# WangWen-Believer/DR-SLAM

Hardware: AMD Instinct MI355X
Metric: RGB-D frames/sec (extract+match) at 640x480 (higher is better)
Workload: dtype u8; 1 GPU; 640x480 synthetic RGB-D (TUM3 intrinsics), ORB extract 1000/1.2/8/20/7 + SearchByProjection(frame k, frame k-1, th=15) on consecutive frames; BASELINE config 2; batch_per_gpu=512, batches_in_flight_per_gpu=3, distinct_resident_input_batches_per_gpu=3, sequence_frames_per_rank=64

## Files before the change

### dr_slam_amd/csrc/capi.cpp

```cpp
#include "drfe_internal.h"
#include "map_upkeep_internal.h"
#include "triangulate_internal.h"
#include "sim3_internal.h"
#include "pnp_internal.h"
#include "init_internal.h"
#include "line3d_internal.h"
#include "pose_opt_internal.h"
#include "trans_opt_internal.h"
#include "sim3_opt_internal.h"
#include <atomic>
#include "post_internal.h"
#include "match_internal.h"
#include "planes_internal.h"
#include "bow_internal.h"
#include "lines_internal.h"

#include <algorithm>
#include <cstdlib>
#include <cstring>
#include <sched.h>
#include <cstdio>
#include <thread>
#include <new>

// ... 77 lines not shown
        hipError_t e = hipDeviceGetStreamPriorityRange(&prLow, &prHigh);
        if (e != hipSuccess) return e;
        static const int split = [] { const char* m = std::getenv("DRFE_LONG_PRIO"); return !m ? 0 : (m[0] == 's' && m[1] == 'p') ? 1 : (m[0] == 'l' ? 2 : 0); }();
        const int mid = (prLow + prHigh) / 2;
        return hipStreamCreateWithPriority(s, hipStreamNonBlocking, (mid != prLow && ((part == 1 && split == 1) || (part == 0 && split == 2))) ? mid : prLow);
    }
    int dev = 0, cus = 0;
    hipError_t e = hipGetDevice(&dev);
    if (e == hipSuccess) e = hipDeviceGetAttribute(&cus, hipDeviceAttributeMultiprocessorCount, dev);
    if (e != hipSuccess) return e;
    std::vector<uint32_t> mask((size_t)(cus + 31) / 32, 0u);
    const int cut = 32 * share / 100;
    for (int i = 0; i < cus; i++) {
        const bool first = (i % 32) < cut;
        if (first == (part == 0)) mask[(size_t)i / 32] |= 1u << (i % 32);
    }
    return hipExtStreamCreateWithCUMask(s, (uint32_t)mask.size(), mask.data());
}

static std::atomic<long long> g_poolCpuNs[3];
void drfe_pool_cpu_add(int pool, long long ns) { if (pool >= 0 && pool < 3) g_poolCpuNs[pool] += ns; }
extern "C" void drfe_debug_pool_cpu_ns(long long* out3) { for (int k = 0; k < 3; k++) out3[k] = g_poolCpuNs[k].exchange(0); }

extern "C" {

const char* drfe_version(void) { return "drfe 0.1 (gfx950)"; }

const char* drfe_last_error(const drfe_ctx* ctx) { return ctx ? ctx->err.c_str() : g_create_err.c_str(); }

void drfe_destroy(drfe_ctx* c)
{
    if (!c) return;
    (void)hipSetDevice(c->device);
    if (c->stream) (void)hipStreamSynchronize(c->stream);
    drfe_match_buffers_free(c);
    drfe_planes_free(c);
    drfe_bow_free(c);
    drfe_lines_free(c);
    drfe_cape_lanes_free(c);
    drfe_manhattan_free(c);
    drfe_plane_match_free(c);
    drfe_map_upkeep_free(c);
    drfe_triangulate_free(c);
    drfe_sim3_free(c);
    drfe_pnp_free(c);
    drfe_init_free(c);
    drfe_line3d_free(c);
    drfe_pose_opt_free(c);
    drfe_trans_opt_free(c);
    drfe_sim3_opt_free(c);
    drfe_post_free(c);
    drfe_one_shot_free(c);
    drfe_frame_lanes_free(c);
    void* ptrs[] = {c->d_geom, c->d_cells, c->d_tiles, c->d_taps, c->d_pattern, c->d_disc, c->d_pyr, c->d_blur,
                    c->d_cand0, c->d_cand1, c->d_node, c->d_candCount, c->d_sel, c->d_selCount, c->d_kps, c->d_kpsUn, c->d_desc,
                    c->d_kpCount, c->d_status, c->d_uRight, c->d_depth, c->d_gridOff, c->d_gridIdx, c->d_cellKp, c->d_cellDesc, c->d_match,
                    c->d_matchCount, c->d_poses, c->d_stage, c->d_callScratch, c->d_kpUV, c->d_kpDepth};
    for (void* p : ptrs)
        if (p) (void)hipFree(p);
    for (int i = 0; i < DRFE_STAGE_COUNT; i++)
        for (int j = 0; j < 2; j++)
            if (c->ev[i][j]) (void)hipEventDestroy(c->ev[i][j]);
    if (c->stream) (void)hipStreamDestroy(c->stream);
    delete c;
}

int drfe_create(const drfe_config* cfg, drfe_ctx** out)
{
    if (!cfg || !out) { g_create_err = "null argument"; return DRFE_ERR_INVALID; }
    *out = nullptr;
    if (cfg->nlevels < 1 || cfg->nlevels > DRFE_MAX_LEVELS || cfg->max_batch < 1 || cfg->nfeatures < 1 ||
        !(cfg->scale_factor > 1.0f) || cfg->max_width < 64 || cfg->max_height < 64 || cfg->max_width > 4095 ||
        cfg->max_height > 4095) {
        g_create_err = "invalid drfe_config";
        return DRFE_ERR_INVALID;
    }
    int ndev = 0;
    if (hipGetDeviceCount(&ndev) != hipSuccess || ndev <= 0) {
        g_create_err = "no HIP device: libdrfe has no CPU path";
        return DRFE_ERR_HIP;
    }
    if (cfg->device < 0 || cfg->device >= ndev) { g_create_err = "device ordinal out of range"; return DRFE_ERR_INVALID; }
    drfe_ctx* c = new (std::nothrow) drfe_ctx();
    if (!c) { g_create_err = "out of host memory"; return DRFE_ERR_INVALID; }
    c->cfg = *cfg;
    c->device = cfg->device;
    c->stream = nullptr;
    c->profile = false;
    c->lastBatch = 0;
    c->glueValid = false;
    c->mb = nullptr;
    c->ps = nullptr;
    c->planeLanes = nullptr;
    c->bow = nullptr;
    c->ls = nullptr;
    c->lsBatch = nullptr;
    c->capeLanes = nullptr;
    c->lsdDeviceGrow = 1;
    c->lsdRectMode = 0;
    c->capeBatch = nullptr;
    c->planesDeviceCape = 1;
    c->lsdDeviceNfa = 1;
    c->lsdStats[0] = c->lsdStats[1] = c->lsdStats[2] = c->lsdStats[3] = 0;
    c->capeStats[0] = c->capeStats[1] = 0;
    c->ahcStats[0] = c->ahcStats[1] = c->ahcStats[2] = c->ahcStats[3] = 0;
    c->planesDeviceVoxel = 1;
    c->planesDeviceRefit = 1;
    c->ahcRefitStats[0] = c->ahcRefitStats[1] = 0;
    c->planesDeviceAhc = 1;
    c->ahcArena = nullptr;
    c->lineWorkers = nullptr;
    c->frameLanes = nullptr;
    c->lineHost = nullptr;
    std::memset(&c->cam, 0, sizeof(c->cam));
    std::memset(&c->geom, 0, sizeof(c->geom));
    std::memset(c->ev, 0, sizeof(c->ev));
    std::memset(c->evUsed, 0, sizeof(c->evUsed));
    c->d_geom = nullptr; c->d_cells = nullptr; c->d_tiles = nullptr; c->d_taps = nullptr; c->d_pattern = nullptr;
    c->d_callScratch = nullptr; c->callScratchBytes = 0;
    c->d_disc = nullptr; c->d_pyr = nullptr; c->d_blur = nullptr; c->d_cand0 = nullptr; c->d_cand1 = nullptr;
    c->d_node = nullptr; c->d_candCount = nullptr; c->d_sel = nullptr; c->d_selCount = nullptr; c->d_kps = nullptr; c->d_kpsUn = nullptr; std::memset(&c->dist, 0, sizeof(c->dist));
    c->d_desc = nullptr; c->d_kpCount = nullptr; c->d_status = nullptr; c->d_uRight = nullptr; c->d_depth = nullptr;
    c->d_gridOff = nullptr; c->d_gridIdx = nullptr; c->d_cellKp = nullptr; c->d_cellDesc = nullptr; c->d_match = nullptr; c->d_matchCount = nullptr;
    c->d_poses = nullptr; c->d_stage = nullptr;

#define CREATE_FAIL(code)                 \
    do {                                  \
        g_create_err = c->err;            \
        drfe_destroy(c);                  \
        return (code);                    \
    } while (0)
#define CHIP(call)                                                                  \
    do {                                                                            \
        hipError_t e__ = (call);                                                    \
        if (e__ != hipSuccess) {                                                    \
            c->err = std::string(#call) + ": " + hipGetErrorString(e__);            \
            CREATE_FAIL(DRFE_ERR_HIP);                                              \
        }                                                                           \
    } while (0)

    CHIP(hipSetDevice(c->device));
    CHIP(hipStreamCreateWithFlags(&c->stream, hipStreamNonBlocking));
    for (int i = 0; i < DRFE_STAGE_COUNT; i++)
        for (int j = 0; j < 2; j++) CHIP(hipEventCreate(&c->ev[i][j]));
    drfe_build_tables(c);
    {
        const char* e = std::getenv("DRFE_FAST_GENERIC");
        c->fastGeneric = (e && e[0] == '1') ? 1 : 0;
        const char* es = std::getenv("DRFE_FAST_SCREEN");
        c->fastScreen = (es && es[0] >= '0' && es[0] <= '2') ? es[0] - '0' : 2;
        c->qtForceN = drfe_quadtree_parse_force(std::getenv("DRFE_QT_FORCE"), c->qtForce);
        const char* el = std::getenv("DRFE_LEVEL0_COPY");
        c->level0Copy = (el && el[0] == '1') ? 1 : 0;
        c->lastInPlace = 0;
        c->level0.assign((size_t)std::max(cfg->max_batch, 1), Level0Record{false, nullptr, 0});
    }

    DevGeom gmax;
    std::memset(&gmax, 0, sizeof(gmax));
    std::vector<FastCell> cells;
    std::vector<BlurTile> tiles;
    std::vector<ResizeTap> taps;
    int rc = drfe_build_geometry(c, cfg->max_width, cfg->max_height, &gmax, &cells, &tiles, &taps);
    if (rc != DRFE_OK) CREATE_FAIL(rc);
    const size_t B = (size_t)cfg->max_batch;
    c->pyrSlotBytesMax = (size_t)gmax.pyrSlotBytes;
    c->blurSlotBytesMax = (size_t)gmax.blurSlotBytes;
    c->candSlotElemsMax = (size_t)gmax.candSlotElems;
    c->maxKp = gmax.kpSlotElems;
    c->cellsCap = (int)cells.size() + 64;
    c->tilesCap = (int)tiles.size() + 64;
    c->tapsCap = (int)taps.size() + 64 + (cfg->nlevels >= 2 ? gmax.lv[1].rzBlocks + 64 : 0);
    const int nl = cfg->nlevels;

    CHIP(dalloc(&c->d_geom, 1));
    CHIP(dalloc(&c->d_cells, (size_t)c->cellsCap));
    CHIP(dalloc(&c->d_tiles, (size_t)c->tilesCap));
    CHIP(dalloc(&c->d_taps, (size_t)c->tapsCap));
    CHIP(dalloc(&c->d_pattern, 1024));
    CHIP(hipMemcpy(c->d_pattern, kPatternHost, 1024, hipMemcpyHostToDevice));
    {
        std::vector<int16_t> disc;
        for (int v = -DRFE_HALF_PATCH; v <= DRFE_HALF_PATCH; v++) {
            const int d = c->umax[v < 0 ? -v : v];
            for (int u = -d; u <= d; u++) { disc.push_back((int16_t)u); disc.push_back((int16_t)v); }
        }
        c->discCount = (int)disc.size() / 2;
        if (c->discCount > 12 * 64) { c->err = "IC_Angle disc exceeds 12 offsets per lane"; CREATE_FAIL(DRFE_ERR_INVALID); }
        CHIP(dalloc(&c->d_disc, disc.size()));
        CHIP(hipMemcpy(c->d_disc, disc.data(), disc.size() * sizeof(int16_t), hipMemcpyHostToDevice));
    }
    CHIP(dalloc(&c->d_pyr, B * c->pyrSlotBytesMax + 256));
    CHIP(dalloc(&c->d_blur, B * c->blurSlotBytesMax));
    CHIP(dalloc(&c->d_cand0, B * c->candSlotElemsMax));
    CHIP(dalloc(&c->d_cand1, B * c->candSlotElemsMax));
    CHIP(dalloc(&c->d_node, B * c->candSlotElemsMax));
    CHIP(dalloc(&c->d_candCount, B * DRFE_CC_SLOT));
    CHIP(dalloc(&c->d_sel, B * (size_t)c->maxKp));
    CHIP(dalloc(&c->d_selCount, B * nl));
    CHIP(dalloc(&c->d_kps, B * (size_t)c->maxKp));
    CHIP(dalloc(&c->d_desc, B * (size_t)c->maxKp * 32));
    CHIP(dalloc(&c->d_kpCount, B));
    CHIP(dalloc(&c->d_status, 4));
    CHIP(dalloc(&c->d_uRight, B * (size_t)c->maxKp));
    CHIP(dalloc(&c->d_depth, B * (size_t)c->maxKp));
    CHIP(dalloc(&c->d_gridOff, B * (DRFE_GRID_CELLS + 1)));
    CHIP(dalloc(&c->d_gridIdx, B * (size_t)c->maxKp));
    CHIP(dalloc(&c->d_cellKp, B * (size_t)c->maxKp));
    CHIP(dalloc(&c->d_cellDesc, B * (size_t)c->maxKp * 2));
    CHIP(dalloc(&c->d_match, B * (size_t)c->maxKp));
    CHIP(dalloc(&c->d_matchCount, B));
    CHIP(dalloc(&c->d_poses, 2 * B * 16));
    c->stageBytes = (size_t)cfg->max_width * cfg->max_height * 2;
    CHIP(dalloc(&c->d_stage, c->stageBytes));
    CHIP(hipMemset(c->d_kpCount, 0, sizeof(int) * B));
    CHIP(hipMemset(c->d_selCount, 0, sizeof(int) * B * nl));
    CHIP(hipMemset(c->d_status, 0, sizeof(int) * 4));
#undef CHIP
#undef CREATE_FAIL
    *out = c;
    return DRFE_OK;
}

int drfe_orb_scale_tables(const drfe_ctx* c, float* scale, float* inv_scale, float* sigma2, float* inv_sigma2)
{
    if (!c) return DRFE_ERR_INVALID;
    for (int i = 0; i < c->cfg.nlevels; i++) {
        if (scale) scale[i] = c->scale[i];
        if (inv_scale) inv_scale[i] = c->invScale[i];
        if (sigma2) sigma2[i] = c->sigma2[i];
        if (inv_sigma2) inv_sigma2[i] = c->invSigma2[i];
    }
    return DRFE_OK;
}

int drfe_orb_max_keypoints(const drfe_ctx* c) { return c ? c->maxKp : DRFE_ERR_INVALID; }

static int check_status(drfe_ctx* c)
{
    int st = 0;
    HIPCHK(c, hipMemcpy(&st, c->d_status, sizeof(int), hipMemcpyDeviceToHost));
    if (st & 1) { c->err = "FAST candidate arena overflow"; return DRFE_ERR_CAPACITY; }
    if (st & 2) { c->err = "quadtree node pool overflow"; return DRFE_ERR_CAPACITY; }
// ... 634 lines not shown
```

### dr_slam_amd/csrc/drfe_internal.h

```cpp
#ifndef DRFE_INTERNAL_H
#define DRFE_INTERNAL_H

#include <hip/hip_runtime.h>
#ifndef DRFE_NO_ROCTX
#include <roctracer/roctx.h>
#else
static inline int roctxRangePushA(const char*) { return 0; }
static inline int roctxRangePop() { return 0; }
#endif
#include <stdint.h>
#include <time.h>
#include <string>
#include <vector>

#include "../../include/drfe.h"
#include "../../include/drfe_debug.h"
#include "hip_buf.h"

#define DRFE_MAX_LEVELS 16
#define DRFE_EDGE 19
#define DRFE_HALF_PATCH 15
#define DRFE_GRID_COLS 64
#define DRFE_GRID_ROWS 48
#define DRFE_GRID_CELLS (DRFE_GRID_COLS * DRFE_GRID_ROWS)
// ... 51 lines not shown
    int inst[DRFE_MAX_LEVELS];
    int nlaunch;
    QtLaunch launch[DRFE_MAX_LEVELS];
};
int drfe_quadtree_design_load(int pixels);
void drfe_quadtree_plan(const DevGeom& g, int nframes, const int* force, int nforce, QtPlan* plan);
int drfe_quadtree_parse_force(const char* text, int* pairs);

#ifndef DRFE_CC_LINE
#define DRFE_CC_LINE 32
#endif
#define DRFE_CC_SLOT (DRFE_MAX_LEVELS * DRFE_CC_LINE)
#define DRFE_CC_IDX(slot, level) ((size_t)(slot) * DRFE_CC_SLOT + (size_t)(level) * DRFE_CC_LINE)

struct FastCell {
    uint16_t x0, y0;
    uint8_t ww, wh;
    uint8_t level, off;
    uint16_t offX, offY;
    uint32_t cellIdx;
    uint32_t srcOff;
    uint32_t pitch;
    uint32_t candOff, candCap;
    uint8_t ncp, nrb, rpl, pad;
    uint32_t ncpMagic;
};

struct BlurTile { uint16_t tx, ty; uint16_t level, pad; };

struct ResizeTap { uint16_t s0, s1; int16_t w0, w1; };

#include "undistort_math.h"
#include "level0_view.h"

struct Level0Record { bool inPlace; const uint8_t* frame; size_t rowStride; };

struct drfe_ctx {
    drfe_config cfg;
    int device;
    hipStream_t stream;
    std::string err;

    std::vector<float> scale, invScale, sigma2, invSigma2;
    std::vector<int> quota;
    int umax[DRFE_HALF_PATCH + 1];
    DevGeom geom;
    int maxKp;

    DevGeom* d_geom;
    FastCell* d_cells; int cellsCap;
    BlurTile* d_tiles; int tilesCap;
    ResizeTap* d_taps; int tapsCap;
    int8_t* d_pattern;
    int16_t* d_disc;
    int discCount;

    uint8_t* d_pyr; size_t pyrSlotBytesMax;
    uint8_t* d_blur; size_t blurSlotBytesMax;
    uint32_t* d_cand0; uint32_t* d_cand1; uint16_t* d_node; size_t candSlotElemsMax;
    int* d_candCount;
    uint32_t* d_sel;
    int* d_selCount;
    drfe_keypoint* d_kps;
    drfe_keypoint* d_kpsUn;
    DrfeDistortion dist;
    uint8_t* d_desc;
    int* d_kpCount;
    int* d_status;
    int fastScreen;
    int fastGeneric;
    int qtForce[2 * DRFE_MAX_LEVELS];
    int qtForceN = 0;
    int level0Copy;
    int lastInPlace;
    bool level0Staged = false;
    std::vector<Level0Record> level0;

    float* d_uRight; float* d_depth;
    int* d_gridOff; int* d_gridIdx;
    uint4* d_cellKp; uint4* d_cellDesc;
    int* d_match; int* d_matchCount;
    float* d_poses;
    uint8_t* d_stage;
    size_t stageBytes;
    uint32_t* d_kpUV;
    uint16_t* d_kpDepth;
    uint8_t* d_callScratch;
    size_t callScratchBytes;

    int lastBatch;
    bool glueValid;
    drfe_camera cam;

    struct MatchBuffers* mb;
    struct PlanesScratch* ps;
    std::vector<struct PlaneLane>* planeLanes;
    struct BowState* bow;
    struct LinesScratch* ls;
    struct LineHost* lineHost;
    struct OrbOneShot* oneShot;
    struct CapeScratch* cape;
    struct CapeBatchArena* capeBatch;
    int planesDeviceCape;
    std::vector<struct CapeLane>* capeLanes;
    struct SnBuffers* sn;
    struct MfBuffers* mf;
    struct PmBuffers* pm;
    struct MuBuffers* mu = nullptr;
// ... 70 lines not shown
    const char* last = static_cast<const char*>(p) + (bytes ? bytes - 1 : 0);
    if (hipPointerGetAttributes(&b, last) != hipSuccess) { (void)hipGetLastError(); return false; }
    return b.type == hipMemoryTypeHost;
}

static inline const char* drfe_stage_name(int stage)
{
    static const char* const names[DRFE_STAGE_COUNT] = {"drfe:pyramid", "drfe:fast", "drfe:quadtree", "drfe:blur", "drfe:orient+desc", "drfe:glue", "drfe:match", "drfe:fast_b"};
    return stage >= 0 && stage < DRFE_STAGE_COUNT ? names[stage] : "drfe:?";
}
static inline void prof_begin(drfe_ctx* c, int stage, hipStream_t s)
{
    (void)roctxRangePushA(drfe_stage_name(stage));
    if (c->profile) { (void)hipEventRecord(c->ev[stage][0], s); c->evUsed[stage] = true; }
}
static inline void prof_end(drfe_ctx* c, int stage, hipStream_t s)
{
    if (c->profile) (void)hipEventRecord(c->ev[stage][1], s);
    (void)roctxRangePop();
}
struct DrfeRange {
    explicit DrfeRange(const char* name) { (void)roctxRangePushA(name); }
    ~DrfeRange() { (void)roctxRangePop(); }
};

static inline hipError_t drfe_event_wait_sleeping(hipEvent_t ev)
{
    for (int spins = 0;; spins++) {
        const hipError_t e = hipEventQuery(ev);
        if (e != hipErrorNotReady) return e;
        if (spins < 4) continue;
        struct timespec ts = {0, spins < 40 ? 20000 : 100000};
        nanosleep(&ts, nullptr);
    }
}

void drfe_pool_cpu_add(int pool, long long ns);
struct DrfePoolCpuScope {
    int pool; struct timespec t0;
    explicit DrfePoolCpuScope(int p) : pool(p) { clock_gettime(CLOCK_THREAD_CPUTIME_ID, &t0); }
    ~DrfePoolCpuScope() { struct timespec t1; clock_gettime(CLOCK_THREAD_CPUTIME_ID, &t1); drfe_pool_cpu_add(pool, (t1.tv_sec - t0.tv_sec) * 1000000000LL + (t1.tv_nsec - t0.tv_nsec)); }
};

hipError_t drfe_long_kernel_stream(hipStream_t* s, int part);

int drfe_default_host_threads();
void drfe_cape_lanes_free(drfe_ctx* c);
void drfe_bow_slot_invalidate(drfe_ctx* c, int slot);
void drfe_bow_slots_invalidate(drfe_ctx* c, int first, int count);
void drfe_one_shot_free(drfe_ctx* c);
void drfe_frame_lanes_free(drfe_ctx* c);

int drfe_build_tables(drfe_ctx* c);
int drfe_build_geometry(drfe_ctx* c, int w, int h, DevGeom* g, std::vector<FastCell>* cells,
                        std::vector<BlurTile>* tiles, std::vector<ResizeTap>* taps);

hipError_t drfe_launch_orb(drfe_ctx* c, const uint8_t* d_gray, size_t frameStride, size_t rowStride, int nframes,
                           hipStream_t s, bool allowInPlace = false);
hipError_t drfe_launch_level0(drfe_ctx* c, const uint8_t* d_gray, size_t frameStride, size_t rowStride, int nframes, hipStream_t s);
void drfe_fastc_list_caps(const DevGeom& g, int caps[2]);
hipError_t drfe_launch_glue(drfe_ctx* c, const uint16_t* d_depth, size_t frameStride, size_t rowStride,
                            const drfe_camera& cam, int nframes, hipStream_t s);
hipError_t drfe_launch_grid(drfe_ctx* c, const drfe_camera& cam, int nframes, hipStream_t s);
hipError_t drfe_launch_kp_pixels(drfe_ctx* c, int nframes, uint32_t* d_uv, hipStream_t s);
hipError_t drfe_launch_match_consecutive(drfe_ctx* c, const drfe_camera& cam, float th, int mono, int checkOri,
                                         int nframes, hipStream_t s);

static inline bool drfe_level0_in_place_ok(const DevGeom& g, const void* d_gray, size_t frameStride, size_t rowStride)
{
    if (!g.l0InPlace || !d_gray) return false;
    if ((((uintptr_t)d_gray | frameStride | rowStride) & 15) != 0) return false;
    if (rowStride < (size_t)g.imgW || rowStride > ((size_t)1 << 20) || (size_t)g.imgH * rowStride >= ((size_t)1 << 31)) return false;
    return true;
}
static inline void drfe_level0_mark_copy(drfe_ctx* c, int first, int count)
{
    for (int s = first; s < first + count && s < (int)c->level0.size(); s++) c->level0[(size_t)s] = Level0Record{false, nullptr, 0};
}

#define DRFE_RESIZE_BLOCK 256
#define DRFE_RESIZE_MAX_FILL 8
#define DRFE_RESIZE_TILE_BYTES 32768
static inline uint32_t drfe_div_magic(uint32_t d) { return d <= 1 ? 0u : (uint32_t)(((1ull << 32) + d - 1) / d); }
#if defined(__HIPCC__)
__device__ __forceinline__ uint32_t drfe_div_by(uint32_t n, uint32_t d, uint32_t magic)
{
    if (!magic) return n;
    uint32_t q = __umulhi(n, magic);
    if (q * d > n) q--;
    return q;
}
__device__ __forceinline__ int drfe_wave_incl_scan(int v, int lane)
{
    v += __builtin_amdgcn_update_dpp(0, v, 0x111, 0xf, 0xf, true);
    v += __builtin_amdgcn_update_dpp(0, v, 0x112, 0xf, 0xf, true);
    v += __builtin_amdgcn_update_dpp(0, v, 0x114, 0xf, 0xf, true);
    v += __builtin_amdgcn_update_dpp(0, v, 0x118, 0xf, 0xf, true);
    const int t0 = __builtin_amdgcn_readlane(v, 15), t1 = __builtin_amdgcn_readlane(v, 31), t2 = __builtin_amdgcn_readlane(v, 47);
    return v + (lane >= 16 ? t0 : 0) + (lane >= 32 ? t1 : 0) + (lane >= 48 ? t2 : 0);
}

__device__ __forceinline__ int drfe_wave_sum_i32(int v)
{
    v += __builtin_amdgcn_update_dpp(0, v, 0xB1, 0xf, 0xf, false);
    v += __builtin_amdgcn_update_dpp(0, v, 0x4E, 0xf, 0xf, false);
    v += __builtin_amdgcn_update_dpp(0, v, 0x124, 0xf, 0xf, false);
// ... 58 lines not shown
```

### dr_slam_amd/csrc/level0_view.h

```cpp
#ifndef DRFE_LEVEL0_VIEW_H
#define DRFE_LEVEL0_VIEW_H

#include <stddef.h>
#include <stdint.h>

#if defined(__HIPCC__)
#define DRFE_L0_HD static __host__ __device__ inline
#else
#define DRFE_L0_HD static inline
#endif

struct Level0Src {
    const uint8_t* base;
    size_t frameStride;
    uint32_t rowStride;
};

DRFE_L0_HD uint32_t drfe_umulhi32(uint32_t a, uint32_t b)
{
#if defined(__HIP_DEVICE_COMPILE__)
    return __umulhi(a, b);
#else
    return (uint32_t)(((uint64_t)a * b) >> 32);
#endif
// ... 1 lines not shown
DRFE_L0_HD uint32_t drfe_divm(uint32_t n, uint32_t d, uint32_t magic)
{
    const uint32_t q = drfe_umulhi32(n, magic);
    return q * d > n ? q - 1 : q;
}

DRFE_L0_HD uint32_t drfe_rz_window_origin(uint32_t s0, uint32_t s1, uint32_t srcPitch) { return s0 * srcPitch + s1; }
DRFE_L0_HD uint32_t drfe_rz_fill_offset(uint32_t j, uint32_t wq, uint32_t wqMagic, uint32_t srcPitch, uint32_t* r, uint32_t* q)
{
    *r = drfe_divm(j, wq, wqMagic);
    *q = j - *r * wq;
    return *r * srcPitch + *q * 16u;
}

DRFE_L0_HD int drfe_l0_fast_off(int x0) { return x0 & 3; }
DRFE_L0_HD uint32_t drfe_l0_fast_origin(int x0, int y0, uint32_t rowStride) { return (uint32_t)y0 * rowStride + (uint32_t)(x0 & ~3); }
DRFE_L0_HD uint32_t drfe_fastc_fill_offset(int i, int nch, uint32_t pitch, int* r, int* c)
{
    *r = nch == 1 ? i : nch == 2 ? (i >> 1) : (int)(((uint32_t)i * 21846u) >> 16);
    *c = i - *r * nch;
#if defined(__HIP_DEVICE_COMPILE__)
    return __umul24((uint32_t)*r, pitch) + (uint32_t)*c * 16u;
#else
    return (uint32_t)*r * pitch + (uint32_t)*c * 16u;
#endif
}

DRFE_L0_HD int drfe_l0_reflect(int p, int n)
{
    if (p < 0) p = -p;
    if (p >= n) p = 2 * (n - 1) - p;
    return p < 0 ? 0 : (p > n - 1 ? n - 1 : p);
}
struct L0BlurCols { uint32_t l, m, r, selL, selR; };
DRFE_L0_HD L0BlurCols drfe_l0_blur_cols(int x, int w)
{
    const int xc = x < w - 4 ? x : w - 4;
    L0BlurCols c;
    c.m = (uint32_t)xc;
    c.l = xc == 0 ? (uint32_t)xc : (uint32_t)(xc - 4);
    c.r = xc == w - 4 ? (uint32_t)xc : (uint32_t)(xc + 4);
    c.selL = xc == 0 ? 0x05060704u : 0x03020100u;
    c.selR = xc == w - 4 ? 0x00000102u : 0x07060504u;
    return c;
}
DRFE_L0_HD uint32_t drfe_l0_blur_row(int y0, int t, int h, uint32_t rowStride) { return (uint32_t)drfe_l0_reflect(y0 + t - 3, h) * rowStride; }

DRFE_L0_HD uint32_t drfe_l0_patch_origin(int x, int y, uint32_t rowStride) { return (uint32_t)(y - 15) * rowStride + (uint32_t)(x - 15); }
DRFE_L0_HD void drfe_desc_raw_dword(int t, int* row, int* colBytes)
{
    *row = (int)(((uint32_t)t * 7282u) >> 16);
    *colBytes = (t - *row * 9) * 4;
}

#endif
```

### dr_slam_amd/csrc/orb_geometry.cpp

```cpp
#include "drfe_internal.h"
#include "../../include/drfe_math.h"

#include <algorithm>
#include <cmath>
#include <cstdlib>

static inline int align_up(int v, int a) { return (v + a - 1) / a * a; }

int drfe_build_tables(drfe_ctx* c)
{
    const int nl = c->cfg.nlevels;
    const double sfd = (double)c->cfg.scale_factor;
    c->scale.assign(nl, 1.f); c->sigma2.assign(nl, 1.f);
    c->invScale.assign(nl, 1.f); c->invSigma2.assign(nl, 1.f);
    for (int i = 1; i < nl; i++) {
        c->scale[i] = (float)(c->scale[i - 1] * sfd);
        c->sigma2[i] = c->scale[i] * c->scale[i];
    }
    for (int i = 0; i < nl; i++) {
        c->invScale[i] = 1.0f / c->scale[i];
        c->invSigma2[i] = 1.0f / c->sigma2[i];
    }
    c->quota.assign(nl, 0);
    const float factor = (float)(1.0f / sfd);
    float want = c->cfg.nfeatures * (1 - factor) / (1 - (float)std::pow((double)factor, (double)nl));
    int sum = 0;
    for (int l = 0; l < nl - 1; l++) {
        c->quota[l] = drfe_round_half_even(want);
        sum += c->quota[l];
        want *= factor;
    }
    c->quota[nl - 1] = std::max(c->cfg.nfeatures - sum, 0);
    const int hp = DRFE_HALF_PATCH;
    for (int v = 0; v <= hp; v++) c->umax[v] = 0;
    const int vmax = (int)std::floor(hp * std::sqrt(2.f) / 2 + 1);
    const int vmin = (int)std::ceil(hp * std::sqrt(2.f) / 2);
    const double hp2 = hp * hp;
    for (int v = 0; v <= vmax; ++v) c->umax[v] = drfe_round_half_even_d(std::sqrt(hp2 - v * v));
    for (int v = hp, v0 = 0; v >= vmin; --v) {
        while (c->umax[v0] == c->umax[v0 + 1]) ++v0;
        c->umax[v] = v0;
        ++v0;
    }
    return DRFE_OK;
}

static void build_taps_axis(int src, int dst, std::vector<ResizeTap>* out)
{
    const double inv = (double)dst / src;
    const double scale = 1. / inv;
    for (int d = 0; d < dst; d++) {
        float f = (float)((d + 0.5) * scale - 0.5);
        int s = (int)std::floor(f);
        f -= s;
        if (s < 0) { s = 0; f = 0; }
        if (s >= src - 1) { s = src - 1; f = 0; }
        ResizeTap t;
        t.s0 = (uint16_t)s;
        t.s1 = (uint16_t)std::min(s + 1, src - 1);
        int w0 = drfe_round_half_even((1.f - f) * 2048.f), w1 = drfe_round_half_even(f * 2048.f);
        t.w0 = (int16_t)std::min(32767, std::max(-32768, w0));
        t.w1 = (int16_t)std::min(32767, std::max(-32768, w1));
        out->push_back(t);
    }
}

static void build_taps(int src, int dst, int padded, std::vector<ResizeTap>* out)
{
    std::vector<ResizeTap> axis;
    build_taps_axis(src, dst, &axis);
    if (out->size() & 1) out->push_back(ResizeTap{0, 0, 0, 0});
    const int bordered = dst + 2 * DRFE_EDGE;
    for (int b = 0; b < padded; b++) {
        if (b >= bordered) { ResizeTap z = out->back(); z.w0 = z.w1 = 0; out->push_back(z); continue; }
        int p = b - DRFE_EDGE;
        if (p < 0) p = -p;
        if (p >= dst) p = 2 * (dst - 1) - p;
        out->push_back(axis[p]);
    }
}

static void plan_resize_tile(DevLevel& L, const DevLevel& P, std::vector<ResizeTap>* taps)
{
    const int bw = L.w + 2 * DRFE_EDGE, bh = L.h + 2 * DRFE_EDGE, B = DRFE_RESIZE_BLOCK;
    const int cols = (bw + 3) / 4;
    int groups = 0, blocks = 0;
    for (int ng = (L.h + 3) / 4; 4 * ng <= bh; ng++) {
        const int nb = (ng * cols + B - 1) / B;
        if (!groups || (long long)ng * cols * blocks > (long long)groups * cols * nb) { groups = ng; blocks = nb; }
    }
    const int extra = 4 * groups - L.h;
    L.rzCols = cols; L.rzGroups = groups; L.rzBlocks = blocks;
    L.rzRow0 = DRFE_EDGE - std::max(0, extra - DRFE_EDGE);
    L.rzColsMagic = drfe_div_magic((uint32_t)cols);
    bool ok = true;
    const ResizeTap* xt = taps->data() + L.xtabOff;
    const ResizeTap* yt = taps->data() + L.ytabOff;
// ... 321 lines not shown
```

### dr_slam_amd/csrc/orb_kernels.hip

```cpp
#include "drfe_internal.h"
#include "../../include/drfe_math.h"

#define WAVE 64

__device__ __forceinline__ int reflect101(int p, int n)
{
    if (p < 0) p = -p;
    if (p >= n) p = 2 * (n - 1) - p;
    return p;
}


#define PYR0_ROWS 2
__global__ __launch_bounds__(256) void k_pyr_level0_wide(const DevLevel L, int pyrSlotBytes, const uint8_t* __restrict__ gray,
                                                         size_t frameStride, size_t rowStride, int x16First, int x16Last,
                                                         uint8_t* __restrict__ pyr)
{
    const int slot = blockIdx.z;
    const int y0 = (blockIdx.y * 4 + threadIdx.y) * PYR0_ROWS;
    const int x16 = x16First + (blockIdx.x * 64 + threadIdx.x) * 16;
    const int bh = L.h + 2 * DRFE_EDGE;
    if (y0 >= bh || x16 > x16Last) return;
    const int sx = x16 - DRFE_EDGE;
    const uint8_t* frame = gray + (size_t)slot * frameStride;
// ... 1014 lines not shown
        };
        for (int p = rr; p < pEnd; p += BLUR_ROWL) {
            uint32_t ha[4], hc[4];
            hsum4raw(drfe_l0_blur_row(y0, 2 * p, h0, src0.rowStride), ha);
            hsum4raw(drfe_l0_blur_row(y0, 2 * p + 1, h0, src0.rowStride), hc);
            *reinterpret_cast<uint4*>(&hb2[p * DRFE_BLUR_TW + cg * 4]) =
                make_uint4(pack16(ha[0], hc[0]), pack16(ha[1], hc[1]), pack16(ha[2], hc[2]), pack16(ha[3], hc[3]));
        }
    } else
    for (int p = rr; p < pEnd; p += BLUR_ROWL) {
        uint32_t ha[4], hc[4];
        const uint32_t ra = (uint32_t)min(y0 + 2 * p - 3 + DRFE_EDGE, lastRow), rc = (uint32_t)min(y0 + 2 * p - 2 + DRFE_EDGE, lastRow);
        hsum4(__umul24(ra, pitch) + col, ha);
        hsum4(__umul24(rc, pitch) + col, hc);
        *reinterpret_cast<uint4*>(&hb2[p * DRFE_BLUR_TW + cg * 4]) =
            make_uint4(pack16(ha[0], hc[0]), pack16(ha[1], hc[1]), pack16(ha[2], hc[2]), pack16(ha[3], hc[3]));
    }
#undef TAP4
    __syncthreads();
    typedef unsigned short u16x2v __attribute__((ext_vector_type(2)));
    const u16x2v t1834 = {18, 34}, t4955 = {49, 55}, t4934 = {49, 34}, t3449 = {34, 49}, t5549 = {55, 49}, t3418 = {34, 18};
    const int blurPitch = L.blurPitch, levelH = L.h;
    if (x0 + cg * 4 >= blurPitch * DRFE_BTILE_W) return;
    uint8_t* base = blur + (size_t)__builtin_amdgcn_readfirstlane(slot) * (size_t)G->blurSlotBytes + (size_t)L.blurOff;
    for (int q = rr; q < DRFE_BLUR_TH / 2; q += BLUR_ROWL) {
        const int y = y0 + 2 * q;
        if (y >= levelH) continue;
        uint4 P[4];
#pragma unroll
        for (int k = 0; k < 4; k++) P[k] = *reinterpret_cast<const uint4*>(&hb2[(q + k) * DRFE_BLUR_TW + cg * 4]);
        uint32_t a[4], c2v[4];
#pragma unroll
        for (int j = 0; j < 4; j++) {
            const uint32_t p0 = (&P[0].x)[j], p1 = (&P[1].x)[j], p2 = (&P[2].x)[j], p3 = (&P[3].x)[j];
            asm("v_mad_u32_u16 %0, %1, 18, %2" : "=v"(a[j]) : "v"(p3), "s"(32768u));
            a[j] = __builtin_amdgcn_udot2(__builtin_bit_cast(u16x2v, p0), t1834, a[j], false);
            a[j] = __builtin_amdgcn_udot2(__builtin_bit_cast(u16x2v, p1), t4955, a[j], false);
            a[j] = __builtin_amdgcn_udot2(__builtin_bit_cast(u16x2v, p2), t4934, a[j], false);
            asm("v_mad_u32_u16 %0, %1, 18, %2 op_sel:[1,0,0,0]" : "=v"(c2v[j]) : "v"(p0), "s"(32768u));
            c2v[j] = __builtin_amdgcn_udot2(__builtin_bit_cast(u16x2v, p1), t3449, c2v[j], false);
            c2v[j] = __builtin_amdgcn_udot2(__builtin_bit_cast(u16x2v, p2), t5549, c2v[j], false);
            c2v[j] = __builtin_amdgcn_udot2(__builtin_bit_cast(u16x2v, p3), t3418, c2v[j], false);
        }
        const uint32_t outA = pack16((uint32_t)__builtin_amdgcn_ashr_pk_u8_i32((int)a[0], (int)a[1], 16),
                                     (uint32_t)__builtin_amdgcn_ashr_pk_u8_i32((int)a[2], (int)a[3], 16));
        const uint32_t outB = pack16((uint32_t)__builtin_amdgcn_ashr_pk_u8_i32((int)c2v[0], (int)c2v[1], 16),
                                     (uint32_t)__builtin_amdgcn_ashr_pk_u8_i32((int)c2v[2], (int)c2v[3], 16));
        *reinterpret_cast<uint32_t*>(base + drfe_blur_offset(x0 + cg * 4, y, blurPitch)) = outA;
        if (y + 1 < levelH) *reinterpret_cast<uint32_t*>(base + drfe_blur_offset(x0 + cg * 4, y + 1, blurPitch)) = outB;
    }
}


#define DESC_DISC_PER_LANE 12
#ifndef DESC_KPW
#define DESC_KPW 4
#endif
#define DESC_REACH 18
#define DESC_RAW_ROWS 31
#define DESC_RAW_DW 9
#define DESC_BLUR_ROWS (2 * DESC_REACH + 1)
#define DESC_BLUR_DW 10
#define DESC_RAW_N (DESC_RAW_ROWS * DESC_RAW_DW)
#define DESC_BLUR_N (DESC_BLUR_ROWS * DESC_BLUR_DW)
#define DESC_RAW_LD 5
#define DESC_BLUR_LD 6
#define DESC_LDS_DW 372
#ifndef DESC_THREADS
#define DESC_THREADS 64
#endif
#define DESC_WAVES (DESC_THREADS / WAVE)
__global__ __launch_bounds__(DESC_THREADS) void k_orient_desc(const DevGeom* __restrict__ G, const uint8_t* __restrict__ pyr,
                                                     const uint8_t* __restrict__ blur,
                                                     const uint32_t* __restrict__ sel,
                                                     const int* __restrict__ selCount,
                                                     const int8_t* __restrict__ pattern,
                                                     const int16_t* __restrict__ disc, int discCount,
                                                     drfe_keypoint* __restrict__ kps, uint8_t* __restrict__ desc,
                                                     int* __restrict__ kpCount, int maxKp, uint32_t gxMagic, const Level0Src src0)
{
    __shared__ uint32_t sPatch[DESC_WAVES][DESC_KPW][DESC_LDS_DW];
    int bx, by;
    drfe_xcd_swizzle_2d(gxMagic, bx, by);
    const int slot = by;
    const int lane = threadIdx.x & (WAVE - 1);
    const int wv = __builtin_amdgcn_readfirstlane((int)(threadIdx.x >> 6));
    const int g0 = (bx * DESC_WAVES + wv) * DESC_KPW;
    const int nl = G->nlevels;
    const int cntL = lane < nl ? selCount[slot * nl + lane] : 0;
    int incl = cntL;
    incl += __builtin_amdgcn_update_dpp(0, incl, 0x111, 0xf, 0xf, true);
    incl += __builtin_amdgcn_update_dpp(0, incl, 0x112, 0xf, 0xf, true);
    incl += __builtin_amdgcn_update_dpp(0, incl, 0x114, 0xf, 0xf, true);
    incl += __builtin_amdgcn_update_dpp(0, incl, 0x118, 0xf, 0xf, true);
    static_assert(DRFE_MAX_LEVELS == 16, "the level prefix assumes one DPP row");
    const int excl = incl - cntL;
    const int total = __builtin_amdgcn_readlane(incl, DRFE_MAX_LEVELS - 1);
    if (g0 == 0 && lane == 0) kpCount[slot] = min(total, maxKp);
    if (g0 >= total || g0 >= maxKp) return;
    int level[DESC_KPW], xi[DESC_KPW], yi[DESC_KPW], resp[DESC_KPW], pitchP[DESC_KPW], pitchB[DESC_KPW];
    int shP[DESC_KPW], shB[DESC_KPW];
    int bx0[DESC_KPW], by0[DESC_KPW];
    bool live[DESC_KPW];
    const uint8_t* cP[DESC_KPW];
    const uint8_t* cB[DESC_KPW];
    uint32_t key[DESC_KPW];
#pragma unroll
    for (int j = 0; j < DESC_KPW; j++) {
        const int g = g0 + j;
        live[j] = g < total && g < maxKp;
        const int lv = live[j] ? __popcll(__ballot(lane < DRFE_MAX_LEVELS && g >= incl)) : 0;
        const int first = __builtin_amdgcn_readlane(excl, lv);
        level[j] = lv;
        key[j] = live[j] ? sel[(size_t)slot * G->kpSlotElems + G->lv[lv].kpOff + (g - first)] : 0u;
    }
#pragma unroll
    for (int j = 0; j < DESC_KPW; j++) {
        const DevLevel& L = G->lv[level[j]];
        xi[j] = (int)(key[j] & 0xFFF) + L.minBX; yi[j] = (int)((key[j] >> 12) & 0xFFF) + L.minBY;
        resp[j] = (int)(key[j] >> 24);
        pitchP[j] = L.pyrPitch; pitchB[j] = L.blurPitch;
        if (!live[j]) { xi[j] = L.minBX + 16; yi[j] = L.minBY + 16; }
        const size_t oP = (size_t)slot * G->pyrSlotBytes + L.pyrOff + (size_t)(yi[j] + DRFE_EDGE - 15) * L.pyrPitch + (xi[j] + DRFE_EDGE - 15);
        shP[j] = (int)(oP & 3); shB[j] = (xi[j] - DESC_REACH) & 3;
        cP[j] = pyr + (oP & ~(size_t)3);
        if (src0.base != nullptr && level[j] == 0) {
            const uint32_t o0 = drfe_l0_patch_origin(xi[j], yi[j], src0.rowStride);
            pitchP[j] = (int)src0.rowStride;
            shP[j] = (int)(o0 & 3u);
            cP[j] = src0.base + (size_t)slot * src0.frameStride + (o0 & ~3u);
        }
        cB[j] = blur + (size_t)slot * G->blurSlotBytes + L.blurOff;
        bx0[j] = (xi[j] - DESC_REACH) & ~3; by0[j] = yi[j] - DESC_REACH;
    }
    uint32_t rw[DESC_KPW][DESC_RAW_LD], bw[DESC_KPW][DESC_BLUR_LD];
    {
        int rRow[DESC_RAW_LD], rCol[DESC_RAW_LD], bRow[DESC_BLUR_LD], bCol[DESC_BLUR_LD];
#pragma unroll
        for (int k = 0; k < DESC_RAW_LD; k++) {
            const int t = min(lane + k * WAVE, DESC_RAW_N - 1);
            drfe_desc_raw_dword(t, &rRow[k], &rCol[k]);
        }
#pragma unroll
        for (int k = 0; k < DESC_BLUR_LD; k++) {
            const int t = min(lane + k * WAVE, DESC_BLUR_N - 1);
            bRow[k] = (int)(__umul24(t, 6554) >> 16); bCol[k] = (t - __mul24(bRow[k], DESC_BLUR_DW)) * 4;
        }
#pragma unroll
        for (int j = 0; j < DESC_KPW; j++) {
#pragma unroll
            for (int k = 0; k < DESC_RAW_LD; k++)
                rw[j][k] = *reinterpret_cast<const uint32_t*>(cP[j] + (uint32_t)(__mul24(rRow[k], pitchP[j]) + rCol[k]));
#pragma unroll
            for (int k = 0; k < DESC_BLUR_LD; k++)
                bw[j][k] = *reinterpret_cast<const uint32_t*>(cB[j] + drfe_blur_offset(bx0[j] + bCol[k], by0[j] + bRow[k], pitchB[j]));
        }
    }
    const uint32_t* disc32 = reinterpret_cast<const uint32_t*>(disc);
    uint32_t uv[DESC_DISC_PER_LANE];
#pragma unroll
    for (int k = 0; k < DESC_DISC_PER_LANE; k++) {
        const int t = lane + k * WAVE;
        uv[k] = t < discCount ? disc32[t] : 0u;
    }
    int m10[DESC_KPW], m01[DESC_KPW];
    {
        int I[DESC_KPW][DESC_DISC_PER_LANE];
        int du[DESC_DISC_PER_LANE], dv[DESC_DISC_PER_LANE];
#pragma unroll
        for (int k = 0; k < DESC_DISC_PER_LANE; k++) { du[k] = (int)(short)(uv[k] & 0xFFFF); dv[k] = (int)(short)(uv[k] >> 16); }
#pragma unroll
        for (int j = 0; j < DESC_KPW; j++)
#pragma unroll
            for (int k = 0; k < DESC_RAW_LD; k++) {
                const int t = lane + k * WAVE;
                if (t < DESC_RAW_N) sPatch[wv][j][t] = rw[j][k];
            }
#pragma unroll
        for (int j = 0; j < DESC_KPW; j++) {
            const uint8_t* pb = reinterpret_cast<const uint8_t*>(sPatch[wv][j]) + shP[j];
#pragma unroll
            for (int k = 0; k < DESC_DISC_PER_LANE; k++) I[j][k] = pb[__mul24(dv[k] + 15, DESC_RAW_DW * 4) + (du[k] + 15)];
        }
#pragma unroll
        for (int j = 0; j < DESC_KPW; j++) {
            m10[j] = 0; m01[j] = 0;
#pragma unroll
            for (int k = 0; k < DESC_DISC_PER_LANE; k++) {
                m10[j] += du[k] * I[j][k];
                m01[j] += dv[k] * I[j][k];
            }
        }
    }
#pragma unroll
    for (int j = 0; j < DESC_KPW; j++) { m10[j] = drfe_wave_sum_i32(m10[j]); m01[j] = drfe_wave_sum_i32(m01[j]); }
    uint32_t pat[4];
#pragma unroll
    for (int r = 0; r < 4; r++) pat[r] = reinterpret_cast<const uint32_t*>(pattern)[r * 64 + lane];
    const float factorPI = (float)(3.1415926535897932384626433832795 / 180.f);
    float angle[DESC_KPW], cosA[DESC_KPW], sinA[DESC_KPW];
    {
        int my01 = 0, my10 = 0;
#pragma unroll
        for (int j = 0; j < DESC_KPW; j++)
            if (lane == j) { my01 = m01[j]; my10 = m10[j]; }
        const float ang = drfe_fast_atan2((float)my01, (float)my10);
        float sn, cs;
        drfe_sincos(ang * factorPI, &sn, &cs);
#pragma unroll
        for (int j = 0; j < DESC_KPW; j++) {
            angle[j] = __builtin_bit_cast(float, __builtin_amdgcn_readlane(__builtin_bit_cast(int, ang), j));
            cosA[j] = __builtin_bit_cast(float, __builtin_amdgcn_readlane(__builtin_bit_cast(int, cs), j));
            sinA[j] = __builtin_bit_cast(float, __builtin_amdgcn_readlane(__builtin_bit_cast(int, sn), j));
        }
    }
#pragma unroll
    for (int j = 0; j < DESC_KPW; j++)
#pragma unroll
        for (int k = 0; k < DESC_BLUR_LD; k++) {
            const int t = lane + k * WAVE;
            if (t < DESC_BLUR_N) sPatch[wv][j][t] = bw[j][k];
        }
    typedef float f32x2 __attribute__((ext_vector_type(2)));
    f32x2 PX[4], PY[4];
#pragma unroll
    for (int r = 0; r < 4; r++) {
        const uint32_t q4 = pat[r];
        PX[r] = f32x2{(float)(int8_t)(q4 & 0xFF), (float)(int8_t)((q4 >> 16) & 0xFF)};
        PY[r] = f32x2{(float)(int8_t)((q4 >> 8) & 0xFF), (float)(int8_t)(q4 >> 24)};
    }
    const f32x2 magic = {12582912.0f, 12582912.0f};
    const uint32_t excess = 0x400000u * (DESC_BLUR_DW * 4) + 0x4B400000u;
    int t0[DESC_KPW][4], t1[DESC_KPW][4];
#pragma unroll
    for (int j = 0; j < DESC_KPW; j++) {
        const f32x2 a = {cosA[j], cosA[j]}, b = {sinA[j], sinA[j]};
        const uint8_t* pc = reinterpret_cast<const uint8_t*>(sPatch[wv][j]) + shB[j] + DESC_REACH * (DESC_BLUR_DW * 4) + DESC_REACH;
#pragma unroll
        for (int r = 0; r < 4; r++) {
            const f32x2 ry = (PX[r] * b + PY[r] * a) + magic;
            const f32x2 rx = (PX[r] * a - PY[r] * b) + magic;
            const float ry0 = ry.x, ry1 = ry.y, rx0 = rx.x, rx1 = rx.y;
            const uint32_t i0 = __umul24(__float_as_uint(ry0), DESC_BLUR_DW * 4) + __float_as_uint(rx0) - excess;
            const uint32_t i1 = __umul24(__float_as_uint(ry1), DESC_BLUR_DW * 4) + __float_as_uint(rx1) - excess;
// ... 91 lines not shown
        }
    }
    prof_end(c, DRFE_STAGE_PYRAMID, s);

    prof_begin(c, DRFE_STAGE_FAST, s);
    if (g.fastCols && !c->fastGeneric) {
        const int nSmall = g.fastColsSmall, nBig = g.totalCells - nSmall;
        if (nSmall > 0)
            hipLaunchKernelGGL((k_fast_cells_cols<8>), dim3(nSmall, nframes), dim3(64), (size_t)fastc_lds_bytes(g.fastColsRows, 8 * 64), s,
                               c->d_cells, g.nlevels, g.pyrSlotBytes, g.candSlotElems, g.iniTh, g.minTh, c->d_pyr, c->d_cand0,
                               c->d_cand1, c->d_candCount, c->d_status, drfe_div_magic((uint32_t)nSmall), 0, c->fastScreen, fastc_list_off(g.fastColsRows), fastc_list_cap(g.fastColsRows, 8 * 64), src0);
        if (nBig > 0) {
            prof_end(c, DRFE_STAGE_FAST, s);
            prof_begin(c, DRFE_STAGE_FAST_B, s);
        }
        if (nBig > 0)
            hipLaunchKernelGGL((k_fast_cells_cols<DRFE_FASTC_MAX_RPL>), dim3(nBig, nframes), dim3(64),
                               (size_t)fastc_lds_bytes(g.fastColsRows, DRFE_FASTC_MAX_RPL * 64), s, c->d_cells, g.nlevels, g.pyrSlotBytes, g.candSlotElems,
                               g.iniTh, g.minTh, c->d_pyr, c->d_cand0, c->d_cand1, c->d_candCount, c->d_status,
                               drfe_div_magic((uint32_t)nBig), nSmall, c->fastScreen, fastc_list_off(g.fastColsRows), fastc_list_cap(g.fastColsRows, DRFE_FASTC_MAX_RPL * 64), src0);
        if (nBig > 0) prof_end(c, DRFE_STAGE_FAST_B, s);
        else prof_end(c, DRFE_STAGE_FAST, s);
    } else {
        hipLaunchKernelGGL(k_fast_cells, dim3(g.totalCells, nframes), dim3(64), (size_t)fast_lds_bytes(g.fastMaxWh), s, c->d_cells,
                           g.nlevels, g.pyrSlotBytes, g.candSlotElems, g.iniTh, g.minTh, c->d_pyr,
                           c->d_cand0, c->d_cand1, c->d_candCount, c->d_status, fast_sc_off(g.fastMaxWh),
                           drfe_div_magic((uint32_t)g.totalCells));
        prof_end(c, DRFE_STAGE_FAST, s);
    }

    prof_begin(c, DRFE_STAGE_QUADTREE, s);
    {
        typedef void (*QtFn)(const DevGeom*, int, const uint32_t*, const uint32_t*, uint16_t*, const int*, uint32_t*, int*, int*);
#define X(T, K, M) k_quadtree<T, K, M>,
        static const QtFn fns[] = {DRFE_QT_INSTANCES(X)};
#undef X
        QtPlan plan;
        drfe_quadtree_plan(g, nframes, c->qtForce, c->qtForceN, &plan);
        for (int i = 0; i < plan.nlaunch; i++) {
            const QtLaunch& q = plan.launch[i];
            hipLaunchKernelGGL(fns[q.inst], dim3(nframes, q.nlevels), dim3(drfe_qt_instances[q.inst].threads), 0, s, c->d_geom, q.level0,
                               c->d_cand0, c->d_cand1, c->d_node, c->d_candCount, c->d_sel, c->d_selCount, c->d_status);
        }
    }
    prof_end(c, DRFE_STAGE_QUADTREE, s);

    prof_begin(c, DRFE_STAGE_BLUR, s);
    hipLaunchKernelGGL(k_blur, dim3(g.totalTiles, nframes), dim3(256), 0, s, c->d_geom, c->d_tiles, c->d_pyr,
                       c->d_blur, drfe_div_magic((uint32_t)g.totalTiles), src0);
    prof_end(c, DRFE_STAGE_BLUR, s);

    prof_begin(c, DRFE_STAGE_DESC, s);
    hipLaunchKernelGGL(k_orient_desc, dim3((c->maxKp + DESC_WAVES * DESC_KPW - 1) / (DESC_WAVES * DESC_KPW), nframes), dim3(DESC_THREADS), 0, s, c->d_geom, c->d_pyr,
                       c->d_blur, c->d_sel, c->d_selCount, c->d_pattern, c->d_disc, c->discCount, c->d_kps,
                       c->d_desc, c->d_kpCount, c->maxKp, drfe_div_magic((uint32_t)((c->maxKp + DESC_WAVES * DESC_KPW - 1) / (DESC_WAVES * DESC_KPW))), src0);
    prof_end(c, DRFE_STAGE_DESC, s);
    return hipGetLastError();
}

size_t drfe_quadtree_lds_bytes() { return sizeof(QtShared<512, DRFE_QT_MAX_NODES>); }

void drfe_fastc_list_caps(const DevGeom& g, int caps[2])
{
    caps[0] = fastc_list_cap(g.fastColsRows, 8 * 64);
    caps[1] = fastc_list_cap(g.fastColsRows, DRFE_FASTC_MAX_RPL * 64);
}
```

Before: 295,800 frames/s.

## Compute IC_Angle moments with udot4 on register-held patch dwords via mask table

Result: no change. 295,200 frames/s (median of 2 runs) (-0.2%).

```diff
diff --git a/dr_slam_amd/csrc/capi.cpp b/dr_slam_amd/csrc/capi.cpp
--- a/dr_slam_amd/csrc/capi.cpp
+++ b/dr_slam_amd/csrc/capi.cpp
@@ -153,7 +153,7 @@
     drfe_post_free(c);
     drfe_one_shot_free(c);
     drfe_frame_lanes_free(c);
-    void* ptrs[] = {c->d_geom, c->d_cells, c->d_tiles, c->d_taps, c->d_pattern, c->d_disc, c->d_pyr, c->d_blur,
+    void* ptrs[] = {c->d_geom, c->d_cells, c->d_tiles, c->d_taps, c->d_pattern, c->d_momIn, c->d_pyr, c->d_blur,
                     c->d_cand0, c->d_cand1, c->d_node, c->d_candCount, c->d_sel, c->d_selCount, c->d_kps, c->d_kpsUn, c->d_desc,
                     c->d_kpCount, c->d_status, c->d_uRight, c->d_depth, c->d_gridOff, c->d_gridIdx, c->d_cellKp, c->d_cellDesc, c->d_match,
                     c->d_matchCount, c->d_poses, c->d_stage, c->d_callScratch, c->d_kpUV, c->d_kpDepth};
@@ -219,7 +219,7 @@
     std::memset(c->evUsed, 0, sizeof(c->evUsed));
     c->d_geom = nullptr; c->d_cells = nullptr; c->d_tiles = nullptr; c->d_taps = nullptr; c->d_pattern = nullptr;
     c->d_callScratch = nullptr; c->callScratchBytes = 0;
-    c->d_disc = nullptr; c->d_pyr = nullptr; c->d_blur = nullptr; c->d_cand0 = nullptr; c->d_cand1 = nullptr;
+    c->d_momIn = nullptr; c->d_pyr = nullptr; c->d_blur = nullptr; c->d_cand0 = nullptr; c->d_cand1 = nullptr;
     c->d_node = nullptr; c->d_candCount = nullptr; c->d_sel = nullptr; c->d_selCount = nullptr; c->d_kps = nullptr; c->d_kpsUn = nullptr; std::memset(&c->dist, 0, sizeof(c->dist));
     c->d_desc = nullptr; c->d_kpCount = nullptr; c->d_status = nullptr; c->d_uRight = nullptr; c->d_depth = nullptr;
     c->d_gridOff = nullptr; c->d_gridIdx = nullptr; c->d_cellKp = nullptr; c->d_cellDesc = nullptr; c->d_match = nullptr; c->d_matchCount = nullptr;
@@ -281,15 +281,11 @@
     CHIP(dalloc(&c->d_pattern, 1024));
     CHIP(hipMemcpy(c->d_pattern, kPatternHost, 1024, hipMemcpyHostToDevice));
     {
-        std::vector<int16_t> disc;
-        for (int v = -DRFE_HALF_PATCH; v <= DRFE_HALF_PATCH; v++) {
-            const int d = c->umax[v < 0 ? -v : v];
-            for (int u = -d; u <= d; u++) { disc.push_back((int16_t)u); disc.push_back((int16_t)v); }
-        }
-        c->discCount = (int)disc.size() / 2;
-        if (c->discCount > 12 * 64) { c->err = "IC_Angle disc exceeds 12 offsets per lane"; CREATE_FAIL(DRFE_ERR_INVALID); }
-        CHIP(dalloc(&c->d_disc, disc.size()));
-        CHIP(hipMemcpy(c->d_disc, disc.data(), disc.size() * sizeof(int16_t), hipMemcpyHostToDevice));
+        std::vector<uint32_t> momW(DRFE_MOMENT_TABLE_DWORDS);
+        drfe_build_moment_table(c->umax, momW.data());
+        const size_t plane = (size_t)DRFE_DESC_RAW_LOADS * 64;
+        CHIP(dalloc(&c->d_momIn, plane));
+        CHIP(hipMemcpy(c->d_momIn, momW.data() + 2 * plane, plane * sizeof(uint32_t), hipMemcpyHostToDevice));
     }
     CHIP(dalloc(&c->d_pyr, B * c->pyrSlotBytesMax + 256));
     CHIP(dalloc(&c->d_blur, B * c->blurSlotBytesMax));
diff --git a/dr_slam_amd/csrc/drfe_internal.h b/dr_slam_amd/csrc/drfe_internal.h
--- a/dr_slam_amd/csrc/drfe_internal.h
+++ b/dr_slam_amd/csrc/drfe_internal.h
@@ -127,8 +127,7 @@
     BlurTile* d_tiles; int tilesCap;
     ResizeTap* d_taps; int tapsCap;
     int8_t* d_pattern;
-    int16_t* d_disc;
-    int discCount;
+    uint32_t* d_momIn;
 
     uint8_t* d_pyr; size_t pyrSlotBytesMax;
     uint8_t* d_blur; size_t blurSlotBytesMax;
@@ -305,6 +304,8 @@
 void drfe_frame_lanes_free(drfe_ctx* c);
 
 int drfe_build_tables(drfe_ctx* c);
+#define DRFE_MOMENT_TABLE_DWORDS (3 * DRFE_DESC_RAW_LOADS * 64)
+void drfe_build_moment_table(const int* umax, uint32_t* out);
 int drfe_build_geometry(drfe_ctx* c, int w, int h, DevGeom* g, std::vector<FastCell>* cells,
                         std::vector<BlurTile>* tiles, std::vector<ResizeTap>* taps);
 
diff --git a/dr_slam_amd/csrc/level0_view.h b/dr_slam_amd/csrc/level0_view.h
--- a/dr_slam_amd/csrc/level0_view.h
+++ b/dr_slam_amd/csrc/level0_view.h
@@ -77,5 +77,17 @@
     *row = (int)(((uint32_t)t * 7282u) >> 16);
     *colBytes = (t - *row * 9) * 4;
 }
+#define DRFE_DESC_RAW_LOADS 5
+#define DRFE_DESC_RAW_DWORDS 279
+DRFE_L0_HD int drfe_desc_raw_slot(int k, int lane)
+{
+    const int t = 63 * k + lane;
+    return lane < 63 && t < DRFE_DESC_RAW_DWORDS ? t : -1;
+}
+DRFE_L0_HD int drfe_desc_raw_fetch(int k, int lane)
+{
+    const int t = 63 * k + lane;
+    return t < DRFE_DESC_RAW_DWORDS - 1 ? t : DRFE_DESC_RAW_DWORDS - 1;
+}
 
 #endif
diff --git a/dr_slam_amd/csrc/orb_geometry.cpp b/dr_slam_amd/csrc/orb_geometry.cpp
--- a/dr_slam_amd/csrc/orb_geometry.cpp
+++ b/dr_slam_amd/csrc/orb_geometry.cpp
@@ -43,6 +43,31 @@
         ++v0;
     }
     return DRFE_OK;
+}
+
+void drfe_build_moment_table(const int* umax, uint32_t* out)
+{
+    for (int k = 0; k < DRFE_DESC_RAW_LOADS; k++)
+        for (int lane = 0; lane < 64; lane++) {
+            uint32_t wu = 0, wv = 0, wm = 0;
+            const int t = drfe_desc_raw_slot(k, lane);
+            if (t >= 0) {
+                int row, colBytes;
+                drfe_desc_raw_dword(t, &row, &colBytes);
+                const int v = row - DRFE_HALF_PATCH;
+                for (int b = 0; b < 4; b++) {
+                    const int u = colBytes + b - DRFE_HALF_PATCH;
+                    const int d = umax[v < 0 ? -v : v];
+                    if (u < -d || u > d) continue;
+                    wu |= (uint32_t)(u + DRFE_HALF_PATCH) << (8 * b);
+                    wv |= (uint32_t)(v + DRFE_HALF_PATCH) << (8 * b);
+                    wm |= 1u << (8 * b);
+                }
+            }
+            out[(0 * DRFE_DESC_RAW_LOADS + k) * 64 + lane] = wu;
+            out[(1 * DRFE_DESC_RAW_LOADS + k) * 64 + lane] = wv;
+            out[(2 * DRFE_DESC_RAW_LOADS + k) * 64 + lane] = wm;
+        }
 }
 
 static void build_taps_axis(int src, int dst, std::vector<ResizeTap>* out)
diff --git a/dr_slam_amd/csrc/orb_kernels.hip b/dr_slam_amd/csrc/orb_kernels.hip
--- a/dr_slam_amd/csrc/orb_kernels.hip
+++ b/dr_slam_amd/csrc/orb_kernels.hip
@@ -1090,7 +1090,6 @@
 }
 
 
-#define DESC_DISC_PER_LANE 12
 #ifndef DESC_KPW
 #define DESC_KPW 4
 #endif
@@ -1104,6 +1103,13 @@
 #define DESC_RAW_LD 5
 #define DESC_BLUR_LD 6
 #define DESC_LDS_DW 372
+static_assert(DESC_RAW_N == DRFE_DESC_RAW_DWORDS && DESC_RAW_LD == DRFE_DESC_RAW_LOADS, "level0_view.h maps the raw patch's dwords to lanes");
+typedef const __attribute__((address_space(1))) uint32_t* desc_global_u32;
+__device__ __forceinline__ uint32_t desc_blur_offset(int x, int y, int tilesX)
+{
+    const uint32_t ux = (uint32_t)x, uy = (uint32_t)y;
+    return (__umul24(uy / DRFE_BTILE_H, (uint32_t)tilesX) + ux / DRFE_BTILE_W) * 128u + (uy % DRFE_BTILE_H) * DRFE_BTILE_W + ux % DRFE_BTILE_W;
+}
 #ifndef DESC_THREADS
 #define DESC_THREADS 64
 #endif
@@ -1113,7 +1119,7 @@
                                                      const uint32_t* __restrict__ sel,
                                                      const int* __restrict__ selCount,
                                                      const int8_t* __restrict__ pattern,
-                                                     const int16_t* __restrict__ disc, int discCount,
+                                                     const uint32_t* __restrict__ momIn,
                                                      drfe_keypoint* __restrict__ kps, uint8_t* __restrict__ desc,
                                                      int* __restrict__ kpCount, int maxKp, uint32_t gxMagic, const Level0Src src0)
 {
@@ -1176,7 +1182,7 @@
         int rRow[DESC_RAW_LD], rCol[DESC_RAW_LD], bRow[DESC_BLUR_LD], bCol[DESC_BLUR_LD];
 #pragma unroll
         for (int k = 0; k < DESC_RAW_LD; k++) {
-            const int t = min(lane + k * WAVE, DESC_RAW_N - 1);
+            const int t = drfe_desc_raw_fetch(k, lane);
             drfe_desc_raw_dword(t, &rRow[k], &rCol[k]);
         }
 #pragma unroll
@@ -1188,46 +1194,42 @@
         for (int j = 0; j < DESC_KPW; j++) {
 #pragma unroll
             for (int k = 0; k < DESC_RAW_LD; k++)
-                rw[j][k] = *reinterpret_cast<const uint32_t*>(cP[j] + (uint32_t)(__mul24(rRow[k], pitchP[j]) + rCol[k]));
+                rw[j][k] = *(desc_global_u32)(cP[j] + (uint32_t)(__mul24(rRow[k], pitchP[j]) + rCol[k]));
+        }
+#pragma unroll
+        for (int j = 0; j < DESC_KPW; j++) {
 #pragma unroll
             for (int k = 0; k < DESC_BLUR_LD; k++)
-                bw[j][k] = *reinterpret_cast<const uint32_t*>(cB[j] + drfe_blur_offset(bx0[j] + bCol[k], by0[j] + bRow[k], pitchB[j]));
-        }
-    }
-    const uint32_t* disc32 = reinterpret_cast<const uint32_t*>(disc);
-    uint32_t uv[DESC_DISC_PER_LANE];
-#pragma unroll
-    for (int k = 0; k < DESC_DISC_PER_LANE; k++) {
-        const int t = lane + k * WAVE;
-        uv[k] = t < discCount ? disc32[t] : 0u;
+                bw[j][k] = *(desc_global_u32)(cB[j] + desc_blur_offset(bx0[j] + bCol[k], by0[j] + bRow[k], pitchB[j]));
+        }
     }
     int m10[DESC_KPW], m01[DESC_KPW];
     {
-        int I[DESC_KPW][DESC_DISC_PER_LANE];
-        int du[DESC_DISC_PER_LANE], dv[DESC_DISC_PER_LANE];
-#pragma unroll
-        for (int k = 0; k < DESC_DISC_PER_LANE; k++) { du[k] = (int)(short)(uv[k] & 0xFFFF); dv[k] = (int)(short)(uv[k] >> 16); }
-#pragma unroll
-        for (int j = 0; j < DESC_KPW; j++)
+        uint32_t wU[DESC_RAW_LD], wV[DESC_RAW_LD], wM[DESC_RAW_LD];
+#pragma unroll
+        for (int k = 0; k < DESC_RAW_LD; k++) {
+            int row, colBytes;
+            drfe_desc_raw_dword(drfe_desc_raw_fetch(k, lane), &row, &colBytes);
+            wM[k] = momIn[k * WAVE + lane];
+            const uint32_t in = (wM[k] << 8) - wM[k];
+            uint32_t cw = (uint32_t)colBytes | ((uint32_t)colBytes << 8), rw2 = (uint32_t)row | ((uint32_t)row << 8);
+            cw |= cw << 16; rw2 |= rw2 << 16;
+            wU[k] = in & (cw + 0x03020100u);
+            wV[k] = in & rw2;
+        }
+#pragma unroll
+        for (int j = 0; j < DESC_KPW; j++) {
+            uint32_t U = 0, V = 0, M = 0;
 #pragma unroll
             for (int k = 0; k < DESC_RAW_LD; k++) {
-                const int t = lane + k * WAVE;
-                if (t < DESC_RAW_N) sPatch[wv][j][t] = rw[j][k];
+                const uint32_t right = (uint32_t)__builtin_amdgcn_update_dpp(0, (int)rw[j][k], FASTC_DPP_SHL, 0xF, 0xF, true);
+                const uint32_t px = __builtin_amdgcn_alignbyte(right, rw[j][k], (uint32_t)shP[j]);
+                U = __builtin_amdgcn_udot4(px, wU[k], U, false);
+                V = __builtin_amdgcn_udot4(px, wV[k], V, false);
+                M = __builtin_amdgcn_udot4(px, wM[k], M, false);
             }
-#pragma unroll
-        for (int j = 0; j < DESC_KPW; j++) {
-            const uint8_t* pb = reinterpret_cast<const uint8_t*>(sPatch[wv][j]) + shP[j];
-#pragma unroll
-            for (int k = 0; k < DESC_DISC_PER_LANE; k++) I[j][k] = pb[__mul24(dv[k] + 15, DESC_RAW_DW * 4) + (du[k] + 15)];
-        }
-#pragma unroll
-        for (int j = 0; j < DESC_KPW; j++) {
-            m10[j] = 0; m01[j] = 0;
-#pragma unroll
-            for (int k = 0; k < DESC_DISC_PER_LANE; k++) {
-                m10[j] += du[k] * I[j][k];
-                m01[j] += dv[k] * I[j][k];
-            }
+            m10[j] = (int)U - 15 * (int)M;
+            m01[j] = (int)V - 15 * (int)M;
         }
     }
 #pragma unroll
@@ -1425,7 +1427,7 @@
 
     prof_begin(c, DRFE_STAGE_DESC, s);
     hipLaunchKernelGGL(k_orient_desc, dim3((c->maxKp + DESC_WAVES * DESC_KPW - 1) / (DESC_WAVES * DESC_KPW), nframes), dim3(DESC_THREADS), 0, s, c->d_geom, c->d_pyr,
-                       c->d_blur, c->d_sel, c->d_selCount, c->d_pattern, c->d_disc, c->discCount, c->d_kps,
+                       c->d_blur, c->d_sel, c->d_selCount, c->d_pattern, c->d_momIn, c->d_kps,
                        c->d_desc, c->d_kpCount, c->maxKp, drfe_div_magic((uint32_t)((c->maxKp + DESC_WAVES * DESC_KPW - 1) / (DESC_WAVES * DESC_KPW))), src0);
     prof_end(c, DRFE_STAGE_DESC, s);
     return hipGetLastError();
```
